# Qi2019KB/UBPL-PoseEstimation

Measured on AMD Instinct MI355X. Metric: images/sec training step (MT_UBPL, 2-stack HG, 256×256) at 1/2/4/8 GPUs; PCK@0.2, higher is better.
Workload: dtype fp32; 1 GPU; MT_UBPL train step, 2 students + 2 EMA teachers, 2 views; model=StackedHourglass HG2 (K=16, AvgPool features), global_batch=32, per_gpu_batch=32, input=256x256x3, heatmap=16x64x64, parallelism=dp1

## Files before the change

ubpl-poseestimation_amd/csrc/conv_split.hip:

```cpp
#include <atomic>
#include "common.h"
#include <cstdlib>
using ubpl::xcd_remap;

typedef float floatx16 __attribute__((ext_vector_type(16)));
typedef float floatx4 __attribute__((ext_vector_type(4)));
typedef __bf16 bf16x8 __attribute__((ext_vector_type(8)));
typedef __bf16 bf16x2 __attribute__((ext_vector_type(2)));
typedef short short8 __attribute__((ext_vector_type(8)));
typedef _Float16 half8 __attribute__((ext_vector_type(8)));

namespace {

#ifndef UBPL_SOL_TEPI
#define UBPL_SOL_TEPI 1
#endif
#ifndef UBPL_PSAH_NA_MAX
#define UBPL_PSAH_NA_MAX 3
#endif
#ifndef UBPL_SOL_LB
#define UBPL_SOL_LB 2
#endif

constexpr int NT = 256;
// ... 1253 lines not shown
            src = dys_m + 2 * ((int64_t)b * Gco * HWp * 16 + ((int64_t)(oh + 1) * Wp + ow0 + 1) * 16);
            plane = dplane;
        } else {
            src = xs_c + 2 * ((int64_t)b * Gci * HWp * 16 + ((int64_t)(oh + kh) * Wp + ow0 + kw_w) * 16);
            plane = xplane;
            base += OB * (1 + kw_w);
        }
#pragma unroll
        for (int p = 0; p < NP; ++p)
#pragma unroll
            for (int gp = 0; gp < 2; ++gp)
                __builtin_amdgcn_global_load_lds((gbl_ptr_t)(src + 2 * p * plane + lane_off[gp]),
                                                 (lds_ptr_t)(base + p * PI + gp * 1024), 16, 0, 0);
    };

    const int g16 = lane >> 4, i16 = lane & 15;
    const int qrow = i16 >> 2, pcol = i16 & 3;
    auto tr_off = [&](int grp, int t) {
        const int row = (8 * (g16 >> 1) + 4 * t + qrow) ^ (4 * (grp & 1));
        return grp * 512 + row * 32 + 8 * pcol;
    };
    int aoffs[2], boffs[TN][2];
#pragma unroll
    for (int t = 0; t < 2; ++t) aoffs[t] = tr_off(wm / 16 + (g16 & 1), t);
#pragma unroll
    for (int j = 0; j < TN; ++j) {
        const int nb = wn / 32 + j;
#pragma unroll
        for (int t = 0; t < 2; ++t) boffs[j][t] = OB * (1 + (nb >> 1)) + tr_off(2 * (nb & 1) + (g16 & 1), t);
    }

    floatx16 acc[TN];
#pragma unroll
    for (int j = 0; j < TN; ++j)
#pragma unroll
        for (int r = 0; r < 16; ++r) acc[j][r] = 0.f;
    const bool bias_wave = kh == bz % 3 && ci0 == 0 && wn == 0;
    float bsum = 0.f;

    if (nkt > 0) stage(0, s_begin);
    if (nkt > 1) stage(1, s_begin + 1);
    for (int t = 0; t < nkt; ++t) {
        if (t + 1 < nkt) vm_wait<2 * NP>();
        else vm_wait<0>();
        __builtin_amdgcn_s_barrier();
        asm volatile("" ::: "memory");
        if (t + 2 < nkt) stage((t + 2) % NS, s_begin + t + 2);
        const char* base = lds + (t % NS) * SB;
        bf16x8 af[NP], bfr[TN][NP];
#pragma unroll
        for (int p = 0; p < NP; ++p) {
            {
                const v4i16 lo = __builtin_amdgcn_ds_read_tr16_b64_v4i16((tr_ptr_t)(base + p * PI + aoffs[0]));
                const v4i16 hi = __builtin_amdgcn_ds_read_tr16_b64_v4i16((tr_ptr_t)(base + p * PI + aoffs[1]));
                const short8 v = {lo[0], lo[1], lo[2], lo[3], hi[0], hi[1], hi[2], hi[3]};
                af[p] = __builtin_bit_cast(bf16x8, v);
            }
#pragma unroll
            for (int j = 0; j < TN; ++j) {
                const v4i16 lo = __builtin_amdgcn_ds_read_tr16_b64_v4i16((tr_ptr_t)(base + p * PI + boffs[j][0]));
                const v4i16 hi = __builtin_amdgcn_ds_read_tr16_b64_v4i16((tr_ptr_t)(base + p * PI + boffs[j][1]));
                const short8 v = {lo[0], lo[1], lo[2], lo[3], hi[0], hi[1], hi[2], hi[3]};
                bfr[j][p] = __builtin_bit_cast(bf16x8, v);
            }
        }
        if (bias_wave) {
#pragma unroll
            for (int p = 0; p < NP; ++p)
#pragma unroll
                for (int e = 0; e < 8; ++e) bsum += piece_elem<NP>(af[p], e);
        }
        floatx16 tmp[TN];
#pragma unroll
        for (int j = 0; j < TN; ++j) tmp[j] = mfma_split0<NP>(af, bfr[j]);
        __builtin_amdgcn_sched_barrier(0);
#pragma unroll
        for (int j = 0; j < TN; ++j) drain(acc[j], tmp[j]);
        asm volatile("s_waitcnt lgkmcnt(0)" ::: "memory");
    }

    float* sl = slab + (int64_t)bz * Cout * Nt;
    const int li = lane & 31, h = lane >> 5;
    float inv = 1.f, binv = 1.f;
    if constexpr (NP == 2) {
        binv = 1.f / *dscale;
        inv = binv / ubpl::FP16_ACT_SCALE;
    }
#pragma unroll
    for (int j = 0; j < TN; ++j) {
        const int nb = wn / 32 + j;
        const int n = (kh * 3 + (nb >> 1)) * Cin + ci0 + 32 * (nb & 1) + li;
#pragma unroll
        for (int r = 0; r < 16; ++r) {
            const int m = m0 + wm + (r & 3) + 8 * (r >> 2) + 4 * h;
            sl[(int64_t)m * Nt + n] = acc[j][r] * inv;
        }
    }
    if (bias_wave) {
        const float v = bsum + __shfl_xor(bsum, 32, 64);
        if (h == 0) sl[(int64_t)(m0 + wm + li) * Nt + Ntot] = v * binv;
    }
}

template <int NP>
__global__ void __launch_bounds__(NT, 2) wgrad_stem_psa_kernel(const uint16_t* __restrict__ dys, int64_t dplane,
                                                              const uint16_t* __restrict__ xs, int64_t xplane,
                                                              int B, int Cout, int H, int W, int steps_per_split,
                                                              float* __restrict__ slab) {
    constexpr int NS = 3, HXP = 19, BROWS = 4 * HXP;
    constexpr int API = 4 * 16 * 32;
    constexpr int BPI = BROWS * 32;
    constexpr int AB = NP * API, SUB = AB + NP * BPI;
    constexpr int AI = NP * 2, BI = NP * 3, NI = AI + BI;
    constexpr int NPW = (NI + 3) / 4;
    __shared__ __attribute__((aligned(16))) char lds[NS * SUB];
    typedef short v4i16 __attribute__((ext_vector_type(4)));
    typedef __attribute__((address_space(3))) v4i16* tr_ptr_t;

    const int Hp = H + 2, Wp = W + 2, Hx = H + 4, Wx = W + 4;
    const int Go = Cout >> 4;
    constexpr int Ntot = 256, Nt = Ntot + 1;
    const int tid = threadIdx.x, lane = tid & 63, wid = __builtin_amdgcn_readfirstlane(tid >> 6);
    const int lam = xcd_remap(blockIdx.x + gridDim.x * blockIdx.y, gridDim.x * gridDim.y);
    const int by = lam % gridDim.x, bz = lam / gridDim.x;
    const int m0 = by * 64;
    const int wsteps = W >> 4;
    const int total_steps = B * H * wsteps;
    const int s_begin = bz * steps_per_split;
    const int s_end = min(total_steps, s_begin + steps_per_split);
    const int nkt = max(0, s_end - s_begin);

    uint32_t loff[NPW];
    int lpiece[NPW];
    bool lisa[NPW], lon[NPW];
    const int lrow = lane >> 1, lhalf = lane & 1;
#pragma unroll
    for (int u = 0; u < NPW; ++u) {
        const int i = u * 4 + wid;
        lon[u] = i < NI;
        lisa[u] = i < AI;
        if (i < AI) {
            const int gl = 2 * (i % 2) + (lrow >> 4);
            const int rphys = lrow & 15, rlog = rphys ^ (4 * (gl & 1));
            lpiece[u] = i / 2;
            loff[u] = (uint32_t)((((int64_t)gl * Hp * Wp) + rlog) * 16 + 8 * lhalf) * 2;
        } else {
            const int j = i - AI, c = j % 3;
            const int q = min(c * 32, BROWS - 32) + lrow;
            const int a = q / HXP, px = q - a * HXP;
            lpiece[u] = j / 3;
            loff[u] = (uint32_t)(((int64_t)a * Wx + px) * 16 + 8 * lhalf) * 2;
        }
    }
    const char* dys_m = reinterpret_cast<const char*>(dys + (int64_t)(m0 >> 4) * Hp * Wp * 16);
    auto stage = [&](int buf, int s) {
        if (s >= s_end) return;
        const int b = s / (H * wsteps);
        const int rem = s - b * (H * wsteps);
        const int oh = rem / wsteps, ow0 = (rem - oh * wsteps) * 16;
        const int64_t aoff = ((int64_t)b * Go * Hp * Wp + (int64_t)(oh + 1) * Wp + ow0 + 1) * 16;
        const int64_t boff = (((int64_t)b * Hx + oh) * Wx + ow0) * 16;
        char* base = lds + buf * SUB;
#pragma unroll
        for (int u = 0; u < NPW; ++u) {
            if (!lon[u]) continue;
            const int i = u * 4 + wid;
            if (lisa[u]) {
                const char* src = dys_m + 2 * (lpiece[u] * dplane + aoff);
                __builtin_amdgcn_global_load_lds((gbl_ptr_t)(src + loff[u]),
                                                 (lds_ptr_t)(base + lpiece[u] * API + (i % 2) * 1024), 16, 0, 0);
            } else {
                const int j = i - AI, c = j % 3;
                const char* src = reinterpret_cast<const char*>(xs) + 2 * (lpiece[u] * xplane + boff);
                __builtin_amdgcn_global_load_lds((gbl_ptr_t)(src + loff[u]),
                                                 (lds_ptr_t)(base + AB + lpiece[u] * BPI + min(c * 32, BROWS - 32) * 32),
                                                 16, 0, 0);
            }
        }
    };
    const int mine = (NI - wid + 3) / 4;

    const int g16 = lane >> 4, i16 = lane & 15;
    const int qrow = i16 >> 2, pcol = i16 & 3;
    int aoffs[2][2], boffs[2][2];
#pragma unroll
    for (int i = 0; i < 2; ++i)
#pragma unroll
        for (int t = 0; t < 2; ++t) {
            const int grp = 2 * i + (g16 & 1);
            const int row = (8 * (g16 >> 1) + 4 * t + qrow) ^ (4 * (grp & 1));
            aoffs[i][t] = grp * 512 + row * 32 + 8 * pcol;
        }
#pragma unroll
    for (int j = 0; j < 2; ++j)
#pragma unroll
        for (int t = 0; t < 2; ++t) {
            const int px = 8 * (g16 >> 1) + 4 * t + qrow + 2 * j + (g16 & 1);
            boffs[j][t] = (wid * HXP + px) * 32 + 8 * pcol;
        }

    floatx16 acc[2][2];
#pragma unroll
    for (int i = 0; i < 2; ++i)
#pragma unroll
        for (int j = 0; j < 2; ++j)
#pragma unroll
            for (int r = 0; r < 16; ++r) acc[i][j][r] = 0.f;
    const bool bias_wave = wid == 0;
    float bsum[2] = {0.f, 0.f};

    stage(0, s_begin);
    stage(1, s_begin + 1);
    for (int t = 0; t < nkt; ++t) {
        if (t + 1 < nkt) {
            if (mine == 4) vm_wait<4>();
            else if (mine == 3) vm_wait<3>();
            else if (mine == 2) vm_wait<2>();
            else vm_wait<1>();
        } else {
            vm_wait<0>();
        }
        __builtin_amdgcn_s_barrier();
        asm volatile("" ::: "memory");
        if (t + 2 < nkt) stage((t + 2) % NS, s_begin + t + 2);
        char* base = lds + (t % NS) * SUB;
        bf16x8 af[2][NP], bfr[2][NP];
#pragma unroll
        for (int p = 0; p < NP; ++p) {
#pragma unroll
            for (int i = 0; i < 2; ++i) {
                const v4i16 lo = __builtin_amdgcn_ds_read_tr16_b64_v4i16((tr_ptr_t)(base + p * API + aoffs[i][0]));
                const v4i16 hi = __builtin_amdgcn_ds_read_tr16_b64_v4i16((tr_ptr_t)(base + p * API + aoffs[i][1]));
                const short8 v = {lo[0], lo[1], lo[2], lo[3], hi[0], hi[1], hi[2], hi[3]};
                af[i][p] = __builtin_bit_cast(bf16x8, v);
            }
#pragma unroll
            for (int j = 0; j < 2; ++j) {
                const v4i16 lo = __builtin_amdgcn_ds_read_tr16_b64_v4i16((tr_ptr_t)(base + AB + p * BPI + boffs[j][0]));
                const v4i16 hi = __builtin_amdgcn_ds_read_tr16_b64_v4i16((tr_ptr_t)(base + AB + p * BPI + boffs[j][1]));
                const short8 v = {lo[0], lo[1], lo[2], lo[3], hi[0], hi[1], hi[2], hi[3]};
                bfr[j][p] = __builtin_bit_cast(bf16x8, v);
            }
        }
        if (bias_wave) {
#pragma unroll
            for (int i = 0; i < 2; ++i)
#pragma unroll
                for (int p = 0; p < NP; ++p)
#pragma unroll
                    for (int e = 0; e < 8; ++e) bsum[i] += (float)af[i][p][e];
        }
        floatx16 tmp[2][2];
#pragma unroll
        for (int i = 0; i < 2; ++i)
#pragma unroll
            for (int j = 0; j < 2; ++j) tmp[i][j] = mfma_split0<NP>(af[i], bfr[j]);
        __builtin_amdgcn_sched_barrier(0);
#pragma unroll
        for (int i = 0; i < 2; ++i)
#pragma unroll
            for (int j = 0; j < 2; ++j) drain(acc[i][j], tmp[i][j]);
        asm volatile("s_waitcnt lgkmcnt(0)" ::: "memory");
    }

    float* sl = slab + (int64_t)bz * Cout * Nt;
    const int li = lane & 31, h = lane >> 5;
#pragma unroll
    for (int j = 0; j < 2; ++j) {
        const int n = 64 * wid + 32 * j + li;
#pragma unroll
        for (int i = 0; i < 2; ++i)
#pragma unroll
            for (int r = 0; r < 16; ++r) {
                const int m = m0 + 32 * i + (r & 3) + 8 * (r >> 2) + 4 * h;
                sl[(int64_t)m * Nt + n] = acc[i][j][r];
            }
    }
    if (bias_wave) {
#pragma unroll
        for (int i = 0; i < 2; ++i) {
            const float v = bsum[i] + __shfl_xor(bsum[i], 32, 64);
            if (h == 0) sl[(int64_t)(m0 + 32 * i + li) * Nt + Ntot] = v;
        }
    }
}

__global__ void __launch_bounds__(256) stem_wgrad_map_kernel(const float* __restrict__ dws,
                                                             const float* __restrict__ dbs, int Cout, int C,
                                                             float* __restrict__ dw, float* __restrict__ db,
                                                             int accumulate) {
    constexpr int KS = 7;
    const int64_t total = (int64_t)Cout * C * KS * KS;
    const int64_t idx = (int64_t)blockIdx.x * 256 + threadIdx.x;
    if (db != nullptr && idx < Cout) db[idx] = accumulate ? db[idx] + dbs[idx] : dbs[idx];
    if (idx >= total) return;
    const int kw = (int)(idx % KS), kh = (int)((idx / KS) % KS);
    const int c = (int)((idx / (KS * KS)) % C), o = (int)(idx / (KS * KS * C));
    const int ph = (kh + 1) & 1, a = (kh + 1 - ph) / 2;
    const int pw = (kw + 1) & 1, bb = (kw + 1 - pw) / 2;
    const float v = dws[(int64_t)o * 256 + (c * 4 + 2 * ph + pw) * 16 + a * 4 + bb];
    dw[idx] = accumulate ? dw[idx] + v : v;
}

template <bool PRO, int NP = 3, int CM = 128, int CN = 128>
__global__ void __launch_bounds__(NT, 2) wgrad1_sol_kernel(const float* __restrict__ dy, const float* __restrict__ x,
                                                          const float* __restrict__ pscale,
                                                          const float* __restrict__ pshift, int B, int Cin, int Cout,
                                                          int P, int steps_per_split, float* __restrict__ slab) {
    constexpr int TM = CM / 64, TN = CN / 64;
    constexpr int PIA = CM * 32, PIB = CN * 32;
    constexpr int OA = NP * PIA;
    constexpr int SB = OA + NP * PIB;
    constexpr int TPA = NT / CM, TPB = NT / CN;
    constexpr int PPA = 16 / TPA, PPB = 16 / TPB;
    constexpr int FA = PPA / 4, FB = PPB / 4;
    __shared__ __attribute__((aligned(16))) char lds[2 * SB];

    const int tid = threadIdx.x, lane = tid & 63, wid = __builtin_amdgcn_readfirstlane(tid >> 6);
    const int wm = (wid >> 1) * (CM / 2), wn = (wid & 1) * (CN / 2);
    const int lam = xcd_remap(blockIdx.x + gridDim.x * (blockIdx.y + gridDim.y * blockIdx.z),
                              gridDim.x * gridDim.y * gridDim.z);
    const int bx = lam % gridDim.x, by = (lam / gridDim.x) % gridDim.y, bz = lam / (gridDim.x * gridDim.y);
    const int m0 = by * CM, c0 = bx * CN;
    const int psteps = P >> 4;
    const int total = B * psteps;
    const int s_begin = bz * steps_per_split;
    const int s_end = min(total, s_begin + steps_per_split);
    const int nkt = max(0, s_end - s_begin);

    const int ra = tid / TPA, qa = tid % TPA, rb = tid / TPB, qb = tid % TPB;
    const float* arow = dy + (int64_t)(m0 + ra) * P + PPA * qa;
    const float* brow = x + (int64_t)(c0 + rb) * P + PPB * qb;
    float sc = 1.f, sh = 0.f;
    if (PRO) {
        sc = pscale[c0 + rb];
        sh = pshift[c0 + rb];
    }
    const int wofa = ra * 32 + 16 * (((PPA * qa) >> 3) ^ ((ra >> 3) & 1)) + 2 * ((PPA * qa) & 7);
    const int wofb = rb * 32 + 16 * (((PPB * qb) >> 3) ^ ((rb >> 3) & 1)) + 2 * ((PPB * qb) & 7);
    auto gload = [&](float4 (&a)[FA], float4 (&b)[FB], int s) {
        const int bb = s / psteps;
        const int p0 = (s - bb * psteps) * 16;
        const float4* a4 = reinterpret_cast<const float4*>(arow + (int64_t)bb * Cout * P + p0);
        const float4* b4 = reinterpret_cast<const float4*>(brow + (int64_t)bb * Cin * P + p0);
#pragma unroll
        for (int f = 0; f < FA; ++f) a[f] = a4[f];
#pragma unroll
        for (int f = 0; f < FB; ++f) b[f] = b4[f];
    };
    float bsum = 0.f;
    auto split_store = [&](int buf, const float4 (&a)[FA], const float4 (&b)[FB]) {
        float va[PPA], vb[PPB];
#pragma unroll
        for (int f = 0; f < FA; ++f) {
            va[4 * f] = a[f].x, va[4 * f + 1] = a[f].y, va[4 * f + 2] = a[f].z, va[4 * f + 3] = a[f].w;
        }
#pragma unroll
        for (int f = 0; f < FB; ++f) {
            vb[4 * f] = b[f].x, vb[4 * f + 1] = b[f].y, vb[4 * f + 2] = b[f].z, vb[4 * f + 3] = b[f].w;
        }
        if constexpr (PPA == 8)
            bsum += ((va[0] + va[1]) + (va[2] + va[3])) + ((va[4] + va[5]) + (va[6] + va[7]));
        else
            bsum += (va[0] + va[1]) + (va[2] + va[3]);
        if (PRO) {
#pragma unroll
            for (int e = 0; e < PPB; ++e) vb[e] = fmaxf(fmaf(vb[e], sc, sh), 0.f);
        }
        uint32_t pa[NP][PPA / 2], pb[NP][PPB / 2];
#pragma unroll
        for (int e = 0; e < PPA / 2; ++e) {
            uint32_t o[NP];
            split2<NP>(va[2 * e], va[2 * e + 1], o);
#pragma unroll
            for (int p = 0; p < NP; ++p) pa[p][e] = o[p];
        }
#pragma unroll
        for (int e = 0; e < PPB / 2; ++e) {
            uint32_t o[NP];
            split2<NP>(vb[2 * e], vb[2 * e + 1], o);
#pragma unroll
            for (int p = 0; p < NP; ++p) pb[p][e] = o[p];
        }
        char* base = lds + buf * SB;
#pragma unroll
        for (int p = 0; p < NP; ++p) {
            if constexpr (PPA == 8)
                *reinterpret_cast<uint4*>(base + p * PIA + wofa) = make_uint4(pa[p][0], pa[p][1], pa[p][2], pa[p][3]);
            else
                *reinterpret_cast<uint2*>(base + p * PIA + wofa) = make_uint2(pa[p][0], pa[p][1]);
            if constexpr (PPB == 8)
                *reinterpret_cast<uint4*>(base + OA + p * PIB + wofb) =
                    make_uint4(pb[p][0], pb[p][1], pb[p][2], pb[p][3]);
            else
                *reinterpret_cast<uint2*>(base + OA + p * PIB + wofb) = make_uint2(pb[p][0], pb[p][1]);
        }
    };

    floatx16 acc[TM][TN];
#pragma unroll
    for (int i = 0; i < TM; ++i)
#pragma unroll
        for (int j = 0; j < TN; ++j)
#pragma unroll
            for (int q = 0; q < 16; ++q) acc[i][j][q] = 0.f;
    const int li = lane & 31, h = lane >> 5;

    float4 cA[FA], cB[FB], nA[FA], nB[FB];
    if (nkt > 0) gload(cA, cB, s_begin);
    if (nkt > 1) gload(nA, nB, s_begin + 1);
    for (int t = 0; t < nkt; ++t) {
        split_store(t & 1, cA, cB);
#pragma unroll
        for (int f = 0; f < FA; ++f) cA[f] = nA[f];
#pragma unroll
        for (int f = 0; f < FB; ++f) cB[f] = nB[f];
        if (t + 2 < nkt) gload(nA, nB, s_begin + t + 2);
        asm volatile("s_waitcnt lgkmcnt(0)" ::: "memory");
        __builtin_amdgcn_s_barrier();
        asm volatile("" ::: "memory");
        const char* base = lds + (t & 1) * SB;
        bf16x8 af[TM][NP], bfr[TN][NP];
#pragma unroll
        for (int i = 0; i < TM; ++i) {
            const int row = wm + 32 * i + li;
#pragma unroll
            for (int p = 0; p < NP; ++p)
                af[i][p] = *reinterpret_cast<const bf16x8*>(base + p * PIA + row * 32 + 16 * (h ^ ((row >> 3) & 1)));
        }
#pragma unroll
        for (int j = 0; j < TN; ++j) {
            const int row = wn + 32 * j + li;
#pragma unroll
            for (int p = 0; p < NP; ++p)
                bfr[j][p] =
                    *reinterpret_cast<const bf16x8*>(base + OA + p * PIB + row * 32 + 16 * (h ^ ((row >> 3) & 1)));
        }
        if constexpr (NP == 1) {
#pragma unroll
            for (int i = 0; i < TM; ++i)
#pragma unroll
                for (int j = 0; j < TN; ++j) mfma_split<NP>(acc[i][j], af[i], bfr[j]);
        } else {
            floatx16 tmp[TM][TN];
#pragma unroll
            for (int i = 0; i < TM; ++i)
#pragma unroll
                for (int j = 0; j < TN; ++j) {
                    tmp[i][j] = mfma_split0<NP>(af[i], bfr[j]);
                }
            __builtin_amdgcn_sched_barrier(0);
#pragma unroll
            for (int i = 0; i < TM; ++i)
#pragma unroll
                for (int j = 0; j < TN; ++j) drain(acc[i][j], tmp[i][j]);
        }
    }

    const int Nt = Cin + 1;
    float* sl = slab + (int64_t)bz * Cout * Nt;
#pragma unroll
    for (int j = 0; j < TN; ++j) {
        const int n = c0 + wn + 32 * j + li;
#pragma unroll
        for (int i = 0; i < TM; ++i)
#pragma unroll
            for (int q = 0; q < 16; ++q) {
                const int m = m0 + wm + 32 * i + (q & 3) + 8 * (q >> 2) + 4 * h;
                sl[(int64_t)m * Nt + n] = acc[i][j][q];
            }
    }
    float bt = bsum + __shfl_xor(bsum, 1, 64);
    if constexpr (TPA == 4) bt += __shfl_xor(bt, 2, 64);
    if (bx == 0 && qa == 0) sl[(int64_t)(m0 + ra) * Nt + Cin] = bt;
}

__global__ void __launch_bounds__(256) split_reduce_kernel(const float* __restrict__ slab, int splits, int Cout, int P,
                                                          int64_t N, const float* __restrict__ bias, const float* res,
                                                          float* y) {
    const int64_t total = (int64_t)Cout * N;
    for (int64_t i = (int64_t)blockIdx.x * blockDim.x + threadIdx.x; i < total; i += (int64_t)gridDim.x * blockDim.x) {
        const int p = (int)(i % P);
        const int64_t t = i / P;
        const int m = (int)(t % Cout);
        const int64_t b = t / Cout;
        const int64_t n = b * P + p;
        float s = 0.f;
        for (int z = 0; z < splits; ++z) s += slab[((int64_t)z * Cout + m) * N + n];
        if (bias) s += bias[m];
        if (res) s += res[i];
        y[i] = s;
    }
}

__global__ void __launch_bounds__(256) split_relayout_kernel(const float* __restrict__ src,
                                                            uint16_t* __restrict__ dst, int64_t plane,
                                                            const int64_t* __restrict__ table, int mode, int np) {
    const int64_t* e = table + (int64_t)blockIdx.y * 5;
    const int64_t so = e[0], dof = e[1];
    const int Cout = (int)e[2], Cin = (int)e[3], T = (int)e[4];
    const int64_t total = (int64_t)Cout * Cin * T;
    for (int64_t i = (int64_t)blockIdx.x * blockDim.x + threadIdx.x; i < total; i += (int64_t)gridDim.x * blockDim.x) {
        int64_t s;
        if (mode == 0) {
            const int G = ubpl::conv_kgroup(Cin);
            const int gi = (int)(i % G);
            const int64_t t1 = i / G;
            const int tap = (int)(t1 % T);
            const int64_t t2 = t1 / T;
            const int cbk = (int)(t2 % (Cin / G));
            const int co = (int)(t2 / (Cin / G));
            s = ((int64_t)co * Cin + cbk * G + gi) * T + tap;
        } else {
            const int G = ubpl::conv_kgroup(Cout);
            const int gi = (int)(i % G);
            const int64_t t1 = i / G;
            const int tap = (int)(t1 % T);
            const int64_t t2 = t1 / T;
            const int cbk = (int)(t2 % (Cout / G));
            const int ci = (int)(t2 / (Cout / G));
            s = ((int64_t)(cbk * G + gi) * Cin + ci) * T + (T - 1 - tap);
        }
        float v = src[so + s];
        if (np == 2) {
            v *= ubpl::fp16_wscale((mode == 0 ? Cin : Cout) * T);
            const _Float16 hv = (_Float16)v;
            dst[dof + i] = __builtin_bit_cast(uint16_t, hv);
            dst[plane + dof + i] = __builtin_bit_cast(uint16_t, (_Float16)(v - (float)hv));
            continue;
        }
        for (int p = 0; p < np; ++p) {
            const __bf16 hv = (__bf16)v;
            dst[(int64_t)p * plane + dof + i] = __builtin_bit_cast(uint16_t, hv);
            v -= (float)hv;
        }
    }
}

struct Plan {
    int bm, splits, kchunk;
};

struct Occ {
    int ncu = 256;
    int f128[2] = {2, 1}, f64[2] = {3, 2};
    int p128[2] = {2, 2}, p64[2] = {3, 2};
};

const Occ& occ_info();

double plan_cost(int64_t tiles, int s, int64_t nsteps, int occ, int ncu, double step_flops, double slab_bytes) {
    const int64_t blocks = tiles * s;
    const int64_t per_cu = (blocks + ncu - 1) / ncu;
    const int64_t r = per_cu < occ ? per_cu : occ;
    const double eff = r >= 2 ? 1.0 : 0.6;
    const int64_t steps = (nsteps + s - 1) / s;
    const double rate = 2.0e12;
    double t = (double)((per_cu + r - 1) / r) * r * (double)(steps + 2) * step_flops / (rate * eff);
    if (s > 1) t += 2.0 * s * slab_bytes / 5e12 + 4e-6;
    return t;
}

Plan fwd_plan(int Cout, int64_t N, int Ktot, int np, bool psa = false) {
    const Occ& d = occ_info();
    const int bk = psa ? 16 : BK;
    const int nkt = (Ktot + bk - 1) / bk;
    static const bool no_splitk = [] {
        const char* e = std::getenv("UBPL_NO_SPLITK");
        return e != nullptr && e[0] == '1';
    }();
    const int maxs = no_splitk ? 1 : (nkt / 2 > 0 ? nkt / 2 : 1);
    Plan best{64, 1, 0};
    double bc = 1e30;
    for (int bm : {128, 64}) {
        if (bm == 128 && Cout <= 64) continue;
        const int64_t tiles = ((Cout + bm - 1) / bm) * ((N + BN - 1) / BN);
        const int occ = psa ? (bm == 128 ? d.p128[np == 3] : d.p64[np == 3])
                            : (bm == 128 ? d.f128[np == 3] : d.f64[np == 3]);
        const double sf = 2.0 * bm * BN * bk;
        int s_best = 1;
        double c_best = plan_cost(tiles, 1, nkt, occ, d.ncu, sf, 4.0 * Cout * N);
        for (int s = 2; s <= maxs; ++s) {
            const double c = plan_cost(tiles, s, nkt, occ, d.ncu, sf, 4.0 * Cout * N);
            if (c < c_best * 0.97) {
                c_best = c;
                s_best = s;
            }
        }
        const double c = c_best / (bm == 128 ? 1.0 : 0.85);
        if (c < bc) {
            bc = c;
            best.bm = bm;
            best.splits = s_best;
        }
    }
    const int steps = (nkt + best.splits - 1) / best.splits;
    best.kchunk = steps * bk;
    best.splits = (nkt + steps - 1) / steps;
    return best;
}

void launch_split_reduce(const float* slab, int splits, int Cout, int P, int64_t N, const float* bias,
                         const float* res, float* y, hipStream_t st);

inline float psa_osc(int np, int ktot, bool dev_act = false) {
    return np == 2 ? ubpl::fp16_wscale(ktot) * (dev_act ? 1.f : ubpl::FP16_ACT_SCALE) : 1.f;
}

template <int BM, int KS, int NP, int BNT, int WGM = 2, int KSUB = 1>
int launch_psa(const uint16_t* xs, int64_t xplane, const uint16_t* wp, int64_t wplane, const float* bias,
               const float* res, float* y, int B, int Cin, int H, int W, int pad, int Cout, const Plan& pl,
               float* slab, float* stat_part, const ubpl::BnBwdEpi& bwd, hipStream_t st,
               const float* ascp = nullptr) {
    const int64_t N = (int64_t)B * H * W;
    dim3 grid((unsigned)((N + BNT - 1) / BNT), (unsigned)((Cout + BM - 1) / BM), (unsigned)pl.splits);
    const bool split = pl.splits > 1;
    const ubpl::BnBwdEpi off{nullptr, nullptr, 0, nullptr};
    const float osc = psa_osc(NP, Cin * KS * KS, ascp != nullptr);
    if constexpr (NP != 2) {
        if (!split && (stat_part || bwd.part)) {
            hipLaunchKernelGGL((conv_psa_kernel<BM, KS, NP, BNT, WGM, true, KSUB>), grid, dim3(NT), 0, st, xs, xplane,
                               wp, wplane, bias, res, y, B, Cin, H, W, pad, Cout, pl.kchunk, nullptr, stat_part, bwd,
                               osc, ascp);
            UBPL_LAUNCH_CHECK();
            return 0;
        }
    }
    hipLaunchKernelGGL((conv_psa_kernel<BM, KS, NP, BNT, WGM, false, KSUB>), grid,
                       dim3(NT), 0, st, xs, xplane, wp, wplane,
                       bias, split ? nullptr : res, y, B, Cin, H, W, pad, Cout, pl.kchunk, split ? slab : nullptr,
                       nullptr, off, osc, ascp);
    UBPL_LAUNCH_CHECK();
    if (split) {
        launch_split_reduce(slab, pl.splits, Cout, H * W, N, bias, res, y, st);
        UBPL_LAUNCH_CHECK();
        if (stat_part) {
            const int e = ubpl_bn_partials(y, B, Cout, H * W, stat_part, st);
            if (e) return e;
        }
        if (bwd.part)
            return ubpl_bn_backward_partials(y, bwd.x, B, Cout, H * W, bwd.coef, bwd.coef + Cout,
                                             bwd.coef + 2 * Cout, bwd.relu, bwd.part, st);
    }
    return 0;
}

template <int BM, int KS, int ST, bool PRO, int NP>
int launch_fwd(const float* x, const uint16_t* wp, int64_t plane, const float* bias, const float* ps, const float* sh,
               const float* res, float* y, int B, int Cin, int H, int W, int Cout, int Ho, int Wo, const Plan& pl,
               float* slab, hipStream_t st) {
    const int64_t N = (int64_t)B * Ho * Wo;
    dim3 grid((unsigned)((N + BN - 1) / BN), (unsigned)((Cout + BM - 1) / BM), (unsigned)pl.splits);
    const bool split = pl.splits > 1;
    hipLaunchKernelGGL((conv_fwd_split_kernel<BM, KS, ST, PRO, NP>), grid, dim3(NT), 0, st, x, wp, plane, bias, ps, sh,
                       split ? nullptr : res, y, B, Cin, H, W, Cout, Ho, Wo, pl.kchunk, split ? slab : nullptr);
    UBPL_LAUNCH_CHECK();
    if (split) {
        launch_split_reduce(slab, pl.splits, Cout, Ho * Wo, N, bias, res, y, st);
        UBPL_LAUNCH_CHECK();
    }
    return 0;
}

void launch_split_reduce(const float* slab, int splits, int Cout, int P, int64_t N, const float* bias,
                         const float* res, float* y, hipStream_t st) {
    const int64_t total = (int64_t)Cout * N;
    int gsz = (int)((total + 255) / 256);
    if (gsz > 8192) gsz = 8192;
    hipLaunchKernelGGL(split_reduce_kernel, dim3(gsz), dim3(256), 0, st, slab, splits, Cout, P, N, bias, res, y);
}

template <int KS, int ST, int NP>
int fwd_dispatch(const Plan& pl, bool pro, const float* x, const uint16_t* wp, int64_t plane, const float* bias,
                 const float* ps, const float* sh, const float* res, float* y, int B, int Cin, int H, int W, int Cout,
                 int Ho, int Wo, float* slab, hipStream_t st) {
#define UBPL_FS(BM_, PRO_)                                                                                        \
    return launch_fwd<BM_, KS, ST, PRO_, NP>(x, wp, plane, bias, ps, sh, res, y, B, Cin, H, W, Cout, Ho, Wo, pl, \
                                             slab, st)
    if (pl.bm == 128) {
        if (pro) UBPL_FS(128, true);
        UBPL_FS(128, false);
    }
    if (pro) UBPL_FS(64, true);
    UBPL_FS(64, false);
#undef UBPL_FS
}

const Occ& occ_info() {
    static Occ d = [] {
        Occ r;
        int dev = 0, v = 0;
        if (hipGetDevice(&dev) == hipSuccess &&
            hipDeviceGetAttribute(&v, hipDeviceAttributeMultiprocessorCount, dev) == hipSuccess && v > 0)
            r.ncu = v;
        auto q = [&](const void* f, int& dst) {
            int o = 0;
            if (hipOccupancyMaxActiveBlocksPerMultiprocessor(&o, f, NT, 0) == hipSuccess && o > 0) dst = o;
        };
        q((const void*)conv_fwd_split_kernel<128, 3, 1, true, 2>, r.f128[0]);
        q((const void*)conv_fwd_split_kernel<128, 3, 1, true, 3>, r.f128[1]);
        q((const void*)conv_fwd_split_kernel<64, 3, 1, true, 2>, r.f64[0]);
        q((const void*)conv_fwd_split_kernel<64, 3, 1, true, 3>, r.f64[1]);
        q((const void*)conv_psa_kernel<128, 3, 2>, r.p128[0]);
        q((const void*)conv_psa_kernel<128, 3, 3>, r.p128[1]);
        q((const void*)conv_psa_kernel<64, 3, 2>, r.p64[0]);
        q((const void*)conv_psa_kernel<64, 3, 3>, r.p64[1]);
        (void)hipGetLastError();
        return r;
    }();
    return d;
}

}

UBPL_API int64_t ubpl_conv2d_forward_split_workspace(int B, int Cin, int Cout, int KS, int Ho, int Wo, int npieces) {
    const int64_t N = (int64_t)B * Ho * Wo;
    const Plan pl = fwd_plan(Cout, N, Cin * KS * KS, npieces);
    return pl.splits > 1 ? (int64_t)pl.splits * Cout * N : 0;
}

UBPL_API int ubpl_conv2d_forward_split(const float* x, int B, int Cin, int H, int W, const uint16_t* wsplit,
                                       int64_t plane, const float* bias, int Cout, int KS, int stride,
                                       const float* pscale, const float* pshift, const float* res, float* y, int Ho,
                                       int Wo, float* slab, int npieces, void* stream) {
    hipStream_t st = (hipStream_t)stream;
    if (Cin % 16 != 0 || stride != 1 || npieces != 3) return (int)hipErrorInvalidValue;
    if ((((uintptr_t)wsplit) & 15) != 0 || (plane % 8) != 0) return (int)hipErrorInvalidValue;
    const bool pro = pscale != nullptr;
    const int64_t N = (int64_t)B * Ho * Wo;
    const Plan pl = fwd_plan(Cout, N, Cin * KS * KS, npieces);
    if (pl.splits > 1 && slab == nullptr) return (int)hipErrorInvalidValue;
#define UBPL_FD(KS_, NP_)                                                                                     \
    return fwd_dispatch<KS_, 1, NP_>(pl, pro, x, wsplit, plane, bias, pscale, pshift, res, y, B, Cin, H, W, \
                                     Cout, Ho, Wo, slab, st)
    if (KS == 1) UBPL_FD(1, 3);
    if (KS == 3) UBPL_FD(3, 3);
#undef UBPL_FD
    return (int)hipErrorInvalidValue;
}

UBPL_API int ubpl_conv_weights_split(const float* src, uint16_t* dst, int64_t plane, const int64_t* table, int nseg,
                                     int mode, int npieces, void* stream) {
    if (nseg <= 0) return 0;
    if (npieces < 1 || npieces > 3) return (int)hipErrorInvalidValue;
    hipLaunchKernelGGL(split_relayout_kernel, dim3(64, nseg), dim3(256), 0, (hipStream_t)stream, src, dst, plane,
                       table, mode, npieces);
    UBPL_LAUNCH_CHECK();
    return 0;
}

UBPL_API int ubpl_split_activation(const float* x, int B, int C, int H, int W, const float* pscale,
                                   const float* pshift, int pad, int npieces, uint16_t* dst, int64_t plane,
                                   uint16_t* dst3, int64_t plane3, void* stream) {
    if (C % 16 != 0 || npieces < 1 || npieces > 3 || pad < 0 || (plane % 8) != 0) return (int)hipErrorInvalidValue;
    if (dst3 != nullptr && (npieces != 2 || (plane3 % 8) != 0)) return (int)hipErrorInvalidValue;
    const int Hp = H + 2 * pad, Wp = W + 2 * pad;
    dim3 grid((unsigned)((Hp * Wp + 255) / 256), (unsigned)(C / 16), (unsigned)B);
    hipStream_t st = (hipStream_t)stream;
    const bool pro = pscale != nullptr;
// ... 531 lines not shown
```

Baseline: 432.0 images/sec.

## Software-pipeline wgrad split kernel, interleaving bf16 splitting with MFMA chains

Restructures the main loop of the split-bf16 weight-gradient kernel so that the fp32-to-multi-bf16 splitting and LDS stores for the next tile are interleaved between the MFMA chains of the current tile, with the accumulator drain deferred by one chain. It uses explicit sched_group_barrier schedules, incremental pointer arithmetic in place of per-step division, and a packed bf16x2 split helper. The aim is to hide VALU conversion and global-load latency behind matrix-core work. In exchange it adds register pressure from double-buffered staging registers, and the schedule is complex and fragile with respect to compiler behaviour.

```diff
diff --git a/ubpl-poseestimation_amd/csrc/conv_split.hip b/ubpl-poseestimation_amd/csrc/conv_split.hip
--- a/ubpl-poseestimation_amd/csrc/conv_split.hip
+++ b/ubpl-poseestimation_amd/csrc/conv_split.hip
@@ -1579,6 +1579,29 @@
     dw[idx] = accumulate ? dw[idx] + v : v;
 }
 
+template <int NP>
+__device__ __forceinline__ void split2_pk(float a, float b, uint32_t (&o)[NP]) {
+#pragma unroll
+    for (int p = 0; p < NP; ++p) {
+        const bf16x2 v = {(__bf16)a, (__bf16)b};
+        o[p] = __builtin_bit_cast(uint32_t, v);
+        if (p + 1 < NP) {
+            a -= __builtin_bit_cast(float, o[p] << 16);
+            b -= __builtin_bit_cast(float, o[p] & 0xffff0000u);
+        }
+    }
+}
+
+template <int G, int NMF, int NV, int NDW, bool FIRST = true>
+__device__ __forceinline__ void gap_schedule() {
+    if constexpr (G < NMF) {
+        __builtin_amdgcn_sched_group_barrier(0x008, 1, 0);
+        if constexpr (G > 0 || FIRST) __builtin_amdgcn_sched_group_barrier(0x002, NV, 0);
+        if constexpr (G == NMF - 1 && NDW > 0) __builtin_amdgcn_sched_group_barrier(0x200, NDW, 0);
+        gap_schedule<G + 1, NMF, NV, NDW, FIRST>();
+    }
+}
+
 template <bool PRO, int NP = 3, int CM = 128, int CN = 128>
 __global__ void __launch_bounds__(NT, 2) wgrad1_sol_kernel(const float* __restrict__ dy, const float* __restrict__ x,
                                                           const float* __restrict__ pscale,
@@ -1615,19 +1638,29 @@
     }
     const int wofa = ra * 32 + 16 * (((PPA * qa) >> 3) ^ ((ra >> 3) & 1)) + 2 * ((PPA * qa) & 7);
     const int wofb = rb * 32 + 16 * (((PPB * qb) >> 3) ^ ((rb >> 3) & 1)) + 2 * ((PPB * qb) & 7);
-    auto gload = [&](float4 (&a)[FA], float4 (&b)[FB], int s) {
-        const int bb = s / psteps;
-        const int p0 = (s - bb * psteps) * 16;
-        const float4* a4 = reinterpret_cast<const float4*>(arow + (int64_t)bb * Cout * P + p0);
-        const float4* b4 = reinterpret_cast<const float4*>(brow + (int64_t)bb * Cin * P + p0);
+    int ls = s_begin, lp = (s_begin % psteps) * 16;
+    int offa = (s_begin / psteps) * Cout * P + lp, offb = (s_begin / psteps) * Cin * P + lp;
+    auto gload_a = [&](float4 (&a)[FA]) {
+        const float4* a4 = reinterpret_cast<const float4*>(arow + offa);
 #pragma unroll
         for (int f = 0; f < FA; ++f) a[f] = a4[f];
+    };
+    auto gload_b = [&](float4 (&b)[FB]) {
+        const float4* b4 = reinterpret_cast<const float4*>(brow + offb);
 #pragma unroll
         for (int f = 0; f < FB; ++f) b[f] = b4[f];
+        const int adv = ls + 1 < s_end ? 16 : 0;
+        const bool wrap = lp + adv == P;
+        ls += adv >> 4;
+        lp = wrap ? 0 : lp + adv;
+        offa += wrap ? adv + (Cout - 1) * P : adv;
+        offb += wrap ? adv + (Cin - 1) * P : adv;
     };
     float bsum = 0.f;
-    auto split_store = [&](int buf, const float4 (&a)[FA], const float4 (&b)[FB]) {
-        float va[PPA], vb[PPB];
+    constexpr int UA = PPA / 2, NU = (PPA + PPB) / 2;
+    float va[PPA], vb[PPB];
+    uint32_t pa[NP][PPA / 2], pb[NP][PPB / 2];
+    auto split_head = [&](const float4 (&a)[FA], const float4 (&b)[FB]) {
 #pragma unroll
         for (int f = 0; f < FA; ++f) {
             va[4 * f] = a[f].x, va[4 * f + 1] = a[f].y, va[4 * f + 2] = a[f].z, va[4 * f + 3] = a[f].w;
@@ -1644,33 +1677,37 @@
 #pragma unroll
             for (int e = 0; e < PPB; ++e) vb[e] = fmaxf(fmaf(vb[e], sc, sh), 0.f);
         }
-        uint32_t pa[NP][PPA / 2], pb[NP][PPB / 2];
-#pragma unroll
-        for (int e = 0; e < PPA / 2; ++e) {
-            uint32_t o[NP];
-            split2<NP>(va[2 * e], va[2 * e + 1], o);
-#pragma unroll
-            for (int p = 0; p < NP; ++p) pa[p][e] = o[p];
-        }
-#pragma unroll
-        for (int e = 0; e < PPB / 2; ++e) {
-            uint32_t o[NP];
-            split2<NP>(vb[2 * e], vb[2 * e + 1], o);
-#pragma unroll
-            for (int p = 0; p < NP; ++p) pb[p][e] = o[p];
-        }
-        char* base = lds + buf * SB;
+    };
+    auto split_unit = [&](int u) {
+        uint32_t o[NP];
+        if (u < UA) {
+            split2_pk<NP>(va[2 * u], va[2 * u + 1], o);
+#pragma unroll
+            for (int p = 0; p < NP; ++p) pa[p][u] = o[p];
+        } else {
+            split2_pk<NP>(vb[2 * (u - UA)], vb[2 * (u - UA) + 1], o);
+#pragma unroll
+            for (int p = 0; p < NP; ++p) pb[p][u - UA] = o[p];
+        }
+    };
+    auto store_a = [&](int buf) {
 #pragma unroll
         for (int p = 0; p < NP; ++p) {
             if constexpr (PPA == 8)
-                *reinterpret_cast<uint4*>(base + p * PIA + wofa) = make_uint4(pa[p][0], pa[p][1], pa[p][2], pa[p][3]);
+                *reinterpret_cast<uint4*>(lds + buf * SB + p * PIA + wofa) =
+                    make_uint4(pa[p][0], pa[p][1], pa[p][2], pa[p][3]);
             else
-                *reinterpret_cast<uint2*>(base + p * PIA + wofa) = make_uint2(pa[p][0], pa[p][1]);
+                *reinterpret_cast<uint2*>(lds + buf * SB + p * PIA + wofa) = make_uint2(pa[p][0], pa[p][1]);
+        }
+    };
+    auto store_b = [&](int buf) {
+#pragma unroll
+        for (int p = 0; p < NP; ++p) {
             if constexpr (PPB == 8)
-                *reinterpret_cast<uint4*>(base + OA + p * PIB + wofb) =
+                *reinterpret_cast<uint4*>(lds + buf * SB + OA + p * PIB + wofb) =
                     make_uint4(pb[p][0], pb[p][1], pb[p][2], pb[p][3]);
             else
-                *reinterpret_cast<uint2*>(base + OA + p * PIB + wofb) = make_uint2(pb[p][0], pb[p][1]);
+                *reinterpret_cast<uint2*>(lds + buf * SB + OA + p * PIB + wofb) = make_uint2(pb[p][0], pb[p][1]);
         }
     };
 
@@ -1683,19 +1720,18 @@
             for (int q = 0; q < 16; ++q) acc[i][j][q] = 0.f;
     const int li = lane & 31, h = lane >> 5;
 
-    float4 cA[FA], cB[FB], nA[FA], nB[FB];
-    if (nkt > 0) gload(cA, cB, s_begin);
-    if (nkt > 1) gload(nA, nB, s_begin + 1);
-    for (int t = 0; t < nkt; ++t) {
-        split_store(t & 1, cA, cB);
-#pragma unroll
-        for (int f = 0; f < FA; ++f) cA[f] = nA[f];
-#pragma unroll
-        for (int f = 0; f < FB; ++f) cB[f] = nB[f];
-        if (t + 2 < nkt) gload(nA, nB, s_begin + t + 2);
-        asm volatile("s_waitcnt lgkmcnt(0)" ::: "memory");
+    constexpr int NC = TM * TN, CH = NP * (NP + 1) / 2;
+    constexpr int NCU = NC > 1 ? NC - 1 : 1;
+    constexpr int UV = NP == 3 ? 11 : 1;
+    constexpr int NV0 = PPA + (PRO ? 2 * PPB : 0);
+    float4 rA[2][FA], rB[2][FB];
+    floatx16 pend = {};
+    auto step = [&](auto par, auto last, int t) {
+        constexpr int E = decltype(par)::value;
+        constexpr bool LAST = decltype(last)::value;
         __builtin_amdgcn_s_barrier();
         asm volatile("" ::: "memory");
+        __builtin_amdgcn_sched_barrier(0);
         const char* base = lds + (t & 1) * SB;
         bf16x8 af[TM][NP], bfr[TN][NP];
 #pragma unroll
@@ -1713,25 +1749,66 @@
                 bfr[j][p] =
                     *reinterpret_cast<const bf16x8*>(base + OA + p * PIB + row * 32 + 16 * (h ^ ((row >> 3) & 1)));
         }
-        if constexpr (NP == 1) {
-#pragma unroll
-            for (int i = 0; i < TM; ++i)
-#pragma unroll
-                for (int j = 0; j < TN; ++j) mfma_split<NP>(acc[i][j], af[i], bfr[j]);
-        } else {
-            floatx16 tmp[TM][TN];
-#pragma unroll
-            for (int i = 0; i < TM; ++i)
-#pragma unroll
-                for (int j = 0; j < TN; ++j) {
-                    tmp[i][j] = mfma_split0<NP>(af[i], bfr[j]);
-                }
+        __builtin_amdgcn_sched_group_barrier(0x100, (TM + TN) * NP, 0);
+        if constexpr (!LAST) {
+            split_head(rA[E], rB[E]);
+            __builtin_amdgcn_sched_group_barrier(0x002, NV0, 0);
+        }
+        floatx16 prev = pend;
+        auto chain = [&](auto kc) {
+            constexpr int K = decltype(kc)::value, i = K / TN, j = K % TN;
+            constexpr int u0 = LAST || K >= NCU ? 0 : K * NU / NCU, u1 = LAST || K >= NCU ? 0 : (K + 1) * NU / NCU;
+            constexpr bool sa = u0 < UA && u1 >= UA, sb = u0 < NU && u1 == NU;
+            if constexpr (NP == 1) {
+                mfma_split<NP>(acc[i][j], af[i], bfr[j]);
+#pragma unroll
+                for (int u = u0; u < u1; ++u) split_unit(u);
+            } else {
+                const floatx16 cur = mfma_split0<NP>(af[i], bfr[j]);
+#pragma unroll
+                for (int u = u0; u < u1; ++u) split_unit(u);
+                drain(acc[K == 0 ? TM - 1 : (K - 1) / TN][K == 0 ? TN - 1 : (K - 1) % TN], prev);
+                prev = cur;
+            }
+            if constexpr (sa) store_a(E);
+            if constexpr (sb) store_b(E);
+            constexpr int nd = NP > 1 ? 16 : 0, nu = (u1 - u0) * UV;
+            constexpr int nv = nu > 0 || CH == 1 ? (nd + nu + CH - 1) / CH + 1 : (nd + CH - 2) / (CH - 1);
+            gap_schedule<0, CH, nv, (sa ? NP : 0) + (sb ? NP : 0), (nu > 0 || CH == 1)>();
             __builtin_amdgcn_sched_barrier(0);
-#pragma unroll
-            for (int i = 0; i < TM; ++i)
-#pragma unroll
-                for (int j = 0; j < TN; ++j) drain(acc[i][j], tmp[i][j]);
-        }
+            if constexpr (sa) gload_a(rA[E]);
+            if constexpr (sb) gload_b(rB[E]);
+            if constexpr (sa || sb) __builtin_amdgcn_sched_barrier(0);
+        };
+        chain(std::integral_constant<int, 0>{});
+        if constexpr (NC > 1) chain(std::integral_constant<int, 1>{});
+        if constexpr (NC > 2) chain(std::integral_constant<int, 2>{});
+        if constexpr (NC > 3) chain(std::integral_constant<int, 3>{});
+        pend = prev;
+        __builtin_amdgcn_sched_barrier(0);
+        if constexpr (!LAST) asm volatile("s_waitcnt lgkmcnt(0)" ::: "memory");
+    };
+    if (nkt > 0) {
+        gload_a(rA[0]);
+        gload_b(rB[0]);
+        gload_a(rA[1]);
+        gload_b(rB[1]);
+        split_head(rA[0], rB[0]);
+#pragma unroll
+        for (int u = 0; u < NU; ++u) split_unit(u);
+        store_a(0);
+        store_b(0);
+        gload_a(rA[0]);
+        gload_b(rB[0]);
+        asm volatile("s_waitcnt lgkmcnt(0)" ::: "memory");
+        int t = 0;
+        for (int g = (nkt - 1) / 2; g > 0; --g) {
+            step(std::integral_constant<int, 1>{}, std::false_type{}, t++);
+            step(std::integral_constant<int, 0>{}, std::false_type{}, t++);
+        }
+        if (t + 1 < nkt) step(std::integral_constant<int, 1>{}, std::false_type{}, t++);
+        step(std::integral_constant<int, 0>{}, std::true_type{}, t);
+        if constexpr (NP > 1) drain(acc[TM - 1][TN - 1], pend);
     }
 
     const int Nt = Cin + 1;
```

Measured after the change: 433.0 images/sec, median of 6. About the same (+0.2%).
